# mit-acl/dpgo_ros

Measured on AMD Instinct MI355X. Metric: ms/RBCD-iteration + iterations-to-1e-6-relcost, sphere2500 5-agent, lower is better.
Workload: dtype f64; 1 GPU; sphere2500.g2o, 5 agents, synchronous round-robin RBCD, RGD(step 0.2, dense preconditioner) + Nesterov (restart 20), r=5, library weighting; mid-run iterations one launch each (k_step_fd: the private part of an agent's preconditioner product formed by the launch before its own, its row products by the one before that), hipGraphs of up to 256 iterations; agents=5, poses_per_agent=500, placement=agent a on rank a % N

## Files before the change

dpgo_ros_amd/capi.py:

```python
import ctypes as C
import os
import sys
import threading

import numpy as np

_HERE = os.path.dirname(os.path.abspath(__file__))
LIB_PATH = os.environ.get("DPGO_HIP_LIB") or os.path.join(_HERE, "libdpgo_hip.so")
_LIB = None


class Measurement(C.Structure):
    _fields_ = [("r1", C.c_int), ("p1", C.c_int), ("r2", C.c_int), ("p2", C.c_int),
                ("R", C.c_double * 9), ("t", C.c_double * 3),
                ("kappa", C.c_double), ("tau", C.c_double), ("weight", C.c_double),
                ("fixed_weight", C.c_int), ("is_known_inlier", C.c_int)]


MEAS_DTYPE = np.dtype([("r1", "<i4"), ("p1", "<i4"), ("r2", "<i4"), ("p2", "<i4"),
                       ("R", "<f8", (9,)), ("t", "<f8", (3,)),
                       ("kappa", "<f8"), ("tau", "<f8"), ("weight", "<f8"),
                       ("fixed_weight", "<i4"), ("is_known_inlier", "<i4")], align=True)
assert MEAS_DTYPE.itemsize == C.sizeof(Measurement)

# ... 818 lines not shown
    def iteration(self):
        return lib().dpgo_team_iteration(self.h)

    def cost(self):
        f = C.c_double()
        _chk(lib().dpgo_team_cost(self.h, C.byref(f)), "team_cost")
        return f.value

    def update_weights(self):
        return _chk(lib().dpgo_team_update_weights(self.h), "team_update_weights")

    def counters(self):
        out = np.zeros(11)
        lib().dpgo_team_get_counters(self.h, _d(out), 11)
        return out

    def stream(self):
        return lib().dpgo_team_stream(self.h)

    def time_kernel(self, agent_id, which, reps=200):
        ms, nbytes = C.c_double(), C.c_double()
        _chk(lib().dpgo_team_time_kernel(self.h, agent_id, which, reps, C.byref(ms), C.byref(nbytes)), "time_kernel")
        return ms.value, nbytes.value

    def global_X(self):
        return np.concatenate([self.agents[i].get_X() for i in self.ids])

    def certificate_apply(self, V, transport=None, owner_of_robot=None):
        N = int(sum(self.agents[i].n for i in self.ids))
        V = np.ascontiguousarray(V, dtype=np.float64).reshape(-1)
# ... 368 lines not shown
```

dpgo_ros_amd/csrc/capi.hip:

```cpp
#include <unistd.h>

#include <atomic>
#include <array>
#include <chrono>
#include <thread>
#include <unordered_map>

#include <mutex>
#include <random>
#include "certify_internal.h"
#include "team_internal.h"

using namespace dpgo;
using namespace dpgo_host;

extern "C" {

const char *dpgo_last_error(void) { return g_err.c_str(); }

void dpgo_default_params(dpgo_params_t *p, int r, int num_robots) {
  std::memset(p, 0, sizeof *p);
  p->d = 3; p->r = r; p->num_robots = num_robots;
  p->method = DPGO_METHOD_RTR;
  p->rgd_stepsize = 1e-3; p->rgd_use_preconditioner = 1;
// ... 77 lines not shown
    int cus = 0;
    if (hipDeviceGetAttribute(&cus, hipDeviceAttributeMultiprocessorCount, device) == hipSuccess) t->num_cus = cus;
    int lds = 0;
    if (hipDeviceGetAttribute(&lds, hipDeviceAttributeMaxSharedMemoryPerBlock, device) == hipSuccess && lds > 0) t->max_lds = lds;
    const char *e3 = std::getenv("DPGO_BAKE_SEL");
    if (e3) t->bake_sel = (e3[0] == '0') ? 0 : 1;
    const char *e4 = std::getenv("DPGO_BAKE_DESC");
    if (e4) t->bake_desc = (e4[0] == '0') ? 0 : 1;
    const char *e2 = std::getenv("DPGO_FUSED_RTR");
    if (e2) t->use_fused_rtr = (e2[0] == '0') ? 0 : 1;
    const char *e5 = std::getenv("DPGO_FUSED_EVAL");
    if (e5) t->use_fused_eval = (e5[0] == '0') ? 0 : 1;
    if (const char *e6 = std::getenv("DPGO_FE_MIN_N")) t->fe_min_n = std::max(32, std::atoi(e6));
    if (const char *e7 = std::getenv("DPGO_FE_CARRY")) t->use_fe_carry = (e7[0] == '0') ? 0 : 1;
    if (const char *e8 = std::getenv("DPGO_FE_DEEP")) t->use_fe_deep = (e8[0] == '0') ? 0 : 1;
    if (const char *e10 = std::getenv("DPGO_REPORT_TAIL")) t->use_report_tail = (e10[0] == '0') ? 0 : 1;
    if (const char *e11 = std::getenv("DPGO_REPORT_PREFETCH")) t->prefetch_reports = (e11[0] == '0') ? 0 : 1;
    if (t->d_nest_all.alloc(3 * std::max(1, num_local)) ||
        hipMemset(t->d_nest_all.p, 0, sizeof(NestState) * 3 * std::max(1, num_local)) != hipSuccess) {
      delete t; set_err("hand-off state allocation failed"); return nullptr;
    }
    *t->h_bar_err = 0;
  }
  for (int k = 0; k < num_local; ++k) {
    auto a = std::make_unique<Agent>();
    a->id = agent_ids[k]; a->local = k; a->mu = p->gnc_init_mu;
    t->id2local[a->id] = k;
    t->ag.push_back(std::move(a));
  }
  return t;
// ... 1318 lines not shown
    auto sel_at = [&](int rep) { return t->sched[(size_t)((it0 + rep) % P)]; };
    NestState *nest_own = t->d_nest_all.p, *nest_fe[2] = {t->d_nest_all.p + na, t->d_nest_all.p + 2 * na};
    launch_nest_pre(cc, SEL_SCHED, -1, na, mn, p.num_robots, p.restart_interval, 1);
    const int total_reps = ((reps + 1) & ~1) + 8;
    reps = total_reps - 8;
    const int fd_m0 = fe_deep_m0(t);
    if (fd_m0 > 0) {
      int nblk_all = 0;
      for (auto &b : t->ag) nblk_all = std::max(nblk_all, (4 * b->n + 7) / 8);
      double *pacc[2] = {t->d_fd_pacc.p, t->d_fd_pacc.p + (size_t)nblk_all * p.r * 256};
      const int s0 = sel_at(0), s1 = sel_at(1), s2 = sel_at(2);
      launch_fd_prime(cc, s0, s1, s2, mn, p.num_robots, p.restart_interval, nest_own);
      launch_fd_open(cc, fd_m0, s0, s1, pacc[0]);
      for (int k = 0; k < total_reps; ++k) {
        if (k == 8) HIPC(hipEventRecord(e0, t->stream));
        const int flags = FD_IN | (k + 1 < total_reps ? FD_P : 0) | (k + 2 < total_reps ? FD_W : 0) | (k + 3 < total_reps ? FD_Y : 0);
        launch_step_fd(cc, fd_m0, sel_at(k), sel_at(k + 1), sel_at(k + 2), sel_at(k + 3), p.rgd_stepsize, p.num_robots,
                       p.restart_interval, k == 0 ? nest_own : nest_fe[k & 1], nest_fe[(k + 1) & 1], k & 1, flags,
                       pacc[k & 1], pacc[(k + 1) & 1]);
      }
    } else
    for (int k = 0; k < total_reps; ++k) {
      if (k == 8) HIPC(hipEventRecord(e0, t->stream));
      launch_step_fe(cc, sel_at(k), sel_at(k + 1), p.rgd_stepsize, p.num_robots, p.restart_interval,
                     k == 0 ? nest_own : nest_fe[k & 1], nest_fe[(k + 1) & 1], k & 1, sel_at(k + 2),
                     fe_carry_flags(t, k, total_reps, it0));
    }
    HIPC(hipEventRecord(e1, t->stream));
    launch_eval_stats(cc, mn, 0, 0, 1, p.num_robots, p.restart_interval, SEL_SCHED, sel_at(total_reps - 1), nest_fe[total_reps & 1]);
    HIPC(hipEventSynchronize(e1));
    HIPC(hipStreamSynchronize(t->stream));
    t->iter += total_reps;
    float ms = 0;
// ... 48 lines not shown
```

dpgo_ros_amd/csrc/dpgo_dev.h:

```cpp
#pragma once
#include <hip/hip_runtime.h>

namespace dpgo {

enum Buf {
  B_X = 0, B_XPREV, B_Y, B_V, B_G,
  B_EGRAD, B_GF, B_Z, B_ETA, B_R0, B_R1, B_D0, B_D1, B_HD,
  B_X2, B_EGRAD2, B_GF2, B_HETA, B_T0, B_T1, B_T2,
  B_XALT, B_ALTPAD_, B_YALT,
  NBUF
};
constexpr int B_CARRY_Y = B_R0, B_CARRY_W = B_R1, B_CARRY_X = B_D0;
constexpr int B_CARRY_G = B_D1;
constexpr int FE_CARRY_IN = 1, FE_CARRY_W = 2, FE_CARRY_Y = 4;
constexpr int FE_MAX_EDGES = 160;
constexpr int B_ALT = B_XALT - B_X;
static_assert(B_YALT - B_Y == B_ALT, "X and Y twins share one displacement");

struct SharedEdgeDev {
  int lpose;
  int slot;
  int src_agent_local;
  int src_frame;
  int src_robot, pad_;
// ... 89 lines not shown
constexpr int PART_C = 2 * MAX_PART * PART_STRIDE;
constexpr int PART_D = 3 * MAX_PART * PART_STRIDE;
constexpr int PART_E = 4 * MAX_PART * PART_STRIDE;
constexpr int PART_TOTAL = 5 * MAX_PART * PART_STRIDE;

constexpr int LOOKAHEAD_MAX_AGENTS = 8;

struct FeBases {
  const double *ybase[LOOKAHEAD_MAX_AGENTS];
  int npose[LOOKAHEAD_MAX_AGENTS];
  double *part[LOOKAHEAD_MAX_AGENTS];
};

constexpr int FD_IN = 1, FD_P = 2, FD_W = 4, FD_Y = 8;
constexpr int FD_STATS = 16, FD_LASTAT = 32;
struct FdNext {
  const double *Md;
  const double *Gd;
  int N4d, nblk_d;
  unsigned char ord_d[32];
  int n_e, soa_w_e, npub_e, pad_;
  const int *soa_col_e;
  const double *soa_val_e;
  const int *pub_index_e;
  const double *Ye;
  double *We, *Xe, *Ge;
  unsigned char ord_e[32];
};

struct TeamDev {
// ... 25 lines not shown
```

dpgo_ros_amd/csrc/kernels.h:

```cpp
#pragma once
#include <hip/hip_runtime.h>
#include "dpgo_dev.h"

namespace dpgo {

struct LaunchCtx {
  int r;
  hipStream_t stream;
  const AgentDev *agents;
  TeamDev *team;
  int ny = 1;
  int dense_max_n = 1 << 30;
  bool any_two_level = false;
  int tl_max_wg = 0;
  const int *host_precond = nullptr;
  const AgentDev *host_agents = nullptr;
  int num_agents = 0;
  bool bake_desc = false;
  const int *up_slots = nullptr;
  const double *up_in = nullptr;
  int up_n0 = 0, up_n1 = 0;
  int max_lds = 160 * 1024;
  int stage_cap = 0;
  const NestState *nest_all = nullptr;
// ... 31 lines not shown
size_t eval_staged_lds_bytes(int r, int cap);
constexpr int EVS_STATIC_LDS = 8 * 1024;
void launch_hess(const LaunchCtx &c, int sel, int max_n, int xb, int egb, int vb, int ob, int poff);
void launch_precond(const LaunchCtx &c, int sel, int max_n, int mode, int xb, int vb, int zb, int sp, int max_inner,
                    double step, int accel, int num_robots, int advance = PADV_NONE, int restart_interval = 1, int ahead = 0);
void launch_eval_stats(const LaunchCtx &c, int max_n, int first, int has_eval, int has_stats, int num_robots,
                       int restart_interval, int eval_sel = SEL_SCHED, int stats_sel = SEL_SCHED, const NestState *nest_copy = nullptr);
bool step_fe_supported(int r);
int step_fe_max_edges();
void launch_step_fe(const LaunchCtx &c, int sel, int next_sel, double step, int num_robots, int restart_interval,
                    const NestState *nest_src, NestState *nest_dst, int parity, int next2_sel = -1, int carry = 0);
int step_fe_carry_max_poses();
int step_fd_pick_m0(int min_private_chunks);
void launch_fd_open(const LaunchCtx &c, int m0, int s0, int s1, double *pacc_out);
void launch_fd_prime(const LaunchCtx &c, int s0, int s1, int s2, int max_n, int num_robots, int restart_interval, const NestState *nest_src);
void launch_step_fd(const LaunchCtx &c, int m0, int sel, int next_sel, int next2_sel, int next3_sel, double step, int num_robots,
                    int restart_interval, const NestState *nest_src, NestState *nest_dst, int parity, int flags,
                    const double *pacc_in, double *pacc_out);
constexpr int LS_MAX_TRIALS = 8;
void launch_ls_trials(const LaunchCtx &c, int sel, int max_n, int dirb, double step0, double shrink, int ntrials);
void launch_ls_cost(const LaunchCtx &c, int sel, int max_n, int dirb, int ntrials);
void launch_ls_apply(const LaunchCtx &c, int sel, int max_n, double step0, double shrink, double sigma, int ntrials, int tail = 0,
                     int num_robots = 1, int restart_interval = 1);
void launch_tcg_hv(const LaunchCtx &c, int sel, int max_n, int sp, int max_inner);
void launch_retract(const LaunchCtx &c, int sel, int max_n, int xb, int eb, double scale, int ob, int guard_state);
void launch_project_raw(const LaunchCtx &c, const double *X, double *out, int n);
void launch_tangent_raw(const LaunchCtx &c, const double *X, const double *V, double *out, int n);
void launch_retract_raw(const LaunchCtx &c, const double *X, const double *E, double *out, int n);
void launch_nest_pre(const LaunchCtx &c, int sel, int only_agent, int num_agents, int max_n, int num_robots,
                     int restart_interval, int fused_restart = 0);
void launch_stats_nest(const LaunchCtx &c, int num_agents, int max_n, int num_robots, int restart_interval);
void launch_nest_post(const LaunchCtx &c, int sel, int max_n, int num_robots, int restart_interval);
// ... 66 lines not shown
```

dpgo_ros_amd/csrc/step_deep.hip:

```cpp
#include "kernel_common.h"
#include <algorithm>

namespace dpgo {

constexpr int FD_KC = 2048;
#ifndef DPGO_FD_HEAD
#define DPGO_FD_HEAD 0
#endif
#ifndef DPGO_FD_GC_LATE
#define DPGO_FD_GC_LATE 0
#endif
#ifndef DPGO_FD_PACC_WT
#define DPGO_FD_PACC_WT 0
#endif
#ifndef DPGO_FD_E_EARLY
#define DPGO_FD_E_EARLY 0
#endif
#ifndef DPGO_FD_KA_PREFETCH
#define DPGO_FD_KA_PREFETCH 1
#endif
constexpr int FD_HEAD = DPGO_FD_HEAD;

enum { FD_SY_C = 0, FD_SY_E, FD_SY_D, FD_SY_F, FD_SY_N, FD_SY_RQ, FD_SY_COUNT = 8 };

// ... 19 lines not shown
template <int R>
__device__ __forceinline__ int fd_pos_off(const unsigned char *ord, int pose) {
  const int ch = pose >> 4;
  int p = 0;
#pragma unroll
  for (int i = 0; i < 32; ++i) p = ((int)ord[i] == ch) ? i : p;
  return p * 64 * R + (pose & 15) * 4 * R;
}

template <int R>
struct FdXn {
  double2 v[3][2 * R];
};

template <int R>
__device__ __forceinline__ void fd_xn_request(const AgentDev &ag, const FeBases &fb, int parity, int ln, FdXn<R> &xr) {
#pragma unroll
  for (int q = 0; q < 3; ++q) {
    {
      unsigned wsel = 0;
#pragma unroll
      for (int k = 0; k < 32; ++k) {
        const unsigned wk = ag.fe_code[(32 * q + k < FE_MAX_EDGES / 2) ? 32 * q + k : FE_MAX_EDGES / 2 - 1];
        wsel = ((ln >> 1) == k) ? wk : wsel;
      }
      const unsigned code = (ln & 1) ? (wsel >> 16) : (wsel & 0xffffu);
      const int sa = (int)(code >> 12), sf = (int)(code & 0xfffu);
      const double *yb = fb.ybase[0];
      int yn = fb.npose[0];
#pragma unroll
      for (int k = 1; k < LOOKAHEAD_MAX_AGENTS; ++k) { yb = (sa == k) ? fb.ybase[k] : yb; yn = (sa == k) ? fb.npose[k] : yn; }
      const double *xp = yb + (parity ? (size_t)B_ALT * 4 * R * yn : (size_t)0) + (size_t)sf * 4 * R;
#pragma unroll
      for (int k = 0; k < 2 * R; ++k) xr.v[q][k] = ld2(xp + 2 * k);
    }
  }
}

template <int R>
__device__ __forceinline__ void fd_xn_to_lds(const AgentDev &ag, int ln, const FdXn<R> &xr, double *Es) {
  constexpr int EPE = 4 * R + 16;
  int nsh = ag.nshared;
  asm volatile("" : "+v"(nsh));
#pragma unroll
  for (int q = 0; q < 3; ++q) {
    if (64 * q < nsh && 64 * q + ln < nsh) {
      double *E = Es + (size_t)(64 * q + ln) * EPE;
#pragma unroll
      for (int k = 0; k < 2 * R; ++k) *reinterpret_cast<double2 *>(E + 2 * k) = xr.v[q][k];
    }
  }
}

struct FdCf {
  static constexpr int TRIPS = FE_MAX_EDGES * 8 / 64;
  double2 v[TRIPS];
};

__device__ __forceinline__ void fd_cf_request(const AgentDev &ag, int ln, FdCf &cr) {
  const int nit = ag.nshared * 8;
#pragma unroll
  for (int j = 0; j < FdCf::TRIPS; ++j) cr.v[j] = ld2(ag.fe_coef + 2 * min(64 * j + ln, nit - 1));
}

// ... 21 lines not shown
  o.restart_next = ((ns.iter + 3) % restart_interval) == 0;
  o.restart_next2 = ((ns.iter + 4) % restart_interval) == 0;
  o.restart_next3 = ((ns.iter + 5) % restart_interval) == 0;
  o.nest_gamma = o.restart_now ? 0.0 : (1.0 + sqrt(1.0 + 4.0 * Nr * Nr * ns.gamma * ns.gamma)) / (2.0 * Nr);
  const double g2 = (1.0 + sqrt(1.0 + 4.0 * Nr * Nr * o.nest_gamma * o.nest_gamma)) / (2.0 * Nr);
  o.ahead_alpha = 1.0 / (g2 * Nr);
  const double gamma_next = o.restart_next ? 0.0 : g2;
  const double g3 = (1.0 + sqrt(1.0 + 4.0 * Nr * Nr * gamma_next * gamma_next)) / (2.0 * Nr);
  o.ahead2_alpha = 1.0 / (g3 * Nr);
  const double gamma_next2 = o.restart_next2 ? 0.0 : g3;
  const double g4 = (1.0 + sqrt(1.0 + 4.0 * Nr * Nr * gamma_next2 * gamma_next2)) / (2.0 * Nr);
  o.ahead3_alpha = 1.0 / (g4 * Nr);
  return o;
}

template <int R, int NC>
struct FdCur {
  double2 mc[NC];
  double pa[R];
};

template <int R, int M0, int NC>
__device__ __forceinline__ void fd_cur_request(const AgentDev &ag, const double *pacc_in, int bx, int nblk, int l, FdCur<R, NC> &cu) {
  const int cg = (l >> 5) & 7, kl = l & 31;
  const int N4 = ag.N4, col = 8 * bx + cg;
  const double *Mc = ag.M + (size_t)((col < N4) ? col : 0) * N4;
#pragma unroll
  for (int i = 0; i < NC; ++i) cu.mc[i] = ld2_nt(Mc + min(2 * kl + 64 * (int)ag.fe_ord[M0 + i], N4 - 2));
#pragma unroll
  for (int a = 0; a < R; ++a) cu.pa[a] = gp(pacc_in)[((size_t)min(bx, nblk - 1) * R + a) * 256 + l];
// ... 37 lines not shown
#elif defined(DPGO_FD_ENDS)
#define FD_TRACE_DECL
#define FD_STAMP(k) do { if ((k) == 0 && blockIdx.x == 100 && threadIdx.x == 256) ag.part[PART_E + 4000 * PART_STRIDE + 64] = (double)wall_clock64(); } while (0)
#define FD_FLUSH() do { if (blockIdx.x == 100 && (threadIdx.x & 63) == 0) ag.part[PART_E + 4000 * PART_STRIDE + (threadIdx.x >> 6) * 16 + 15] = (double)wall_clock64(); } while (0)
#else
#define FD_TRACE_DECL
#define FD_STAMP(k) do { } while (0)
#define FD_FLUSH() do { } while (0)
#endif

template <int R, int M0>
__global__ __launch_bounds__(512) void k_step_fd(TeamDev *team, int sel, int next_sel, double step, int num_robots, int restart_interval,
                                                 const NestState *nest_src, NestState *nest_dst, int parity, const AgentDev agv,
                                                 int next3_sel, int flags, const FdNext nx, const FeBases fb,
                                                 const double *__restrict__ pacc_in, double *__restrict__ pacc_out, int nblk_all,
                                                 int num_agents) {
  const AgentDev &ag = agv;
#if DPGO_FD_KA_PREFETCH
  {
    const unsigned *ka = (const unsigned *)__builtin_amdgcn_kernarg_segment_ptr();
    constexpr int KA_LINES = (int)((sizeof(AgentDev) + sizeof(FdNext) + sizeof(FeBases) + 160 + 63) / 64);
    unsigned touch = 0;
#pragma unroll
    for (int i = 0; i < KA_LINES; ++i) touch |= ka[16 * i];
    asm volatile("" ::"s"(touch));
  }
#endif
  const double *__restrict__ Xr = ag.buf[parity ? B_XALT : B_X];
  const double *__restrict__ Yr = ag.buf[parity ? B_YALT : B_Y];
  double *__restrict__ Xw = ag.buf[parity ? B_X : B_XALT];
  double *__restrict__ Yw = ag.buf[parity ? B_Y : B_YALT];
// ... 233 lines not shown
    }
    fd_wait(&sy[FD_SY_F], 4);
    if (ln < 8 * R) {
      double s = 0;
#pragma unroll
      for (int q = 0; q < 32; ++q) s += red[q * (8 * R + 1) + ln];
      zs[ln] = s;
    }
    FD_STAMP(6);
    WSYNC();
    const FdNest nn = fd_nest(ns, num_robots, restart_interval);
    const bool restart_now = nn.restart_now, restart_next = nn.restart_next;
    const double nest_gamma = nn.nest_gamma, ahead_alpha = nn.ahead_alpha;
    const bool ahead_opt = next_sel == sel;
    const bool stats = in && (flags & FD_STATS) != 0, lastat = in && (flags & FD_LASTAT) != 0;
    if (ln < 2) tl_rel[ln] = 0.0;
    {
      const int lp = ln >> 4, s = ln & 15;
      if (lp < npose) {
        const size_t o = (size_t)(lp ? pj1 : pj0) * 4 * R;
        double *xs = tl_x + lp * 4 * R, *vsv = tl_v + lp * 4 * R, *ys = tl_y + lp * 4 * R, *Ss = tl_s + lp * 16;
        double *zz = zs + lp * 4 * R;
        const double *x0 = Ysh + lp * 4 * R, *v0 = Esh[0] + lp * 4 * R, *y0 = Esh[1] + lp * 4 * R;
        const int i0 = s, i1 = s + 16;
        const bool h0 = i0 < 4 * R, h1 = i1 < 4 * R;
        tangent_lanes<R>(x0, zz, Ss, s);
        if (h0) xs[i0] = x0[i0] - step * zz[i0];
        if (h1) xs[i1] = x0[i1] - step * zz[i1];
        lanes_sync();
        qf_lanes<R>(xs, Ss, s);
// ... 30 lines not shown
          if (h0 && in) {
            Xw[o + i0] = xs[i0];
            if (!ahead_opt) { Yw[o + i0] = xs[i0]; vsv[i0] = xs[i0]; }
            else Yw[o + i0] = reset ? xs[i0] : y0[i0];
          }
          if (h1 && in) {
            Xw[o + i1] = xs[i1];
            if (!ahead_opt) { Yw[o + i1] = xs[i1]; vsv[i1] = xs[i1]; }
            else Yw[o + i1] = reset ? xs[i1] : y0[i1];
          }
          if (lastat && !ahead_opt && s == 0) gp(ag.part)[PART_D + (lp ? pj1 : pj0)] = 0.0;
        } else {
          if (h0) ys[i0] = (1.0 - ahead_alpha) * xs[i0] + ahead_alpha * vsv[i0];
          if (h1) ys[i1] = (1.0 - ahead_alpha) * xs[i1] + ahead_alpha * vsv[i1];
          lanes_sync();
          polar_lanes<R>(ys, Ss, s);
          FD_STAMP(9);
          if (h0 && in) { Yw[o + i0] = ys[i0]; Xw[o + i0] = ys[i0]; }
          if (h1 && in) { Yw[o + i1] = ys[i1]; Xw[o + i1] = ys[i1]; }
          if (lastat && !ahead_opt && s == 0) {
            double rel2 = 0;
#pragma unroll
            for (int i = 0; i < 4 * R; ++i) { const double d = ys[i] - xs[i]; rel2 += d * d; }
            gp(ag.part)[PART_D + (lp ? pj1 : pj0)] = rel2;
          }
        }
        lanes_sync();
        if (h0 && in) ag.buf[B_V][o + i0] = vsv[i0];
        if (h1 && in) ag.buf[B_V][o + i1] = vsv[i1];
      }
    }
    if (stats) {
      WSYNC();
      double rl = (ln < npose) ? tl_rel[ln] : 0.0;
      rl = wave_sum(rl);
      if (ln == 0 && own) gp(ag.part)[PART_B + (size_t)bx * PART_STRIDE + 2] = rl;
    }
    FD_STAMP(15);
    FD_FLUSH();
    return;
  }

  const int h = cwv - 6;
  if (h == 0) {
    FdXn<R> er;
    fd_xn_request<R>(ag, fb, parity, ln, er);
    FD_STAMP(9);
    FdCur<R, NC> cu;
    fd_cur_request<R, M0, NC>(ag, pacc_in, bx, nblk, tid - 256, cu);
    FD_STAMP(10);
    fd_signal_requested(&sy[FD_SY_RQ]);
    FD_STAMP(11);
    __builtin_amdgcn_s_setprio(3);
    fd_xn_to_lds<R>(ag, ln, er, Es);
    fd_signal(&sy[FD_SY_E]);
    FD_STAMP(8);
    fd_wait(&sy[FD_SY_D], 2);
    fd_cur_product<R, M0, NC>(cu, vs, red, tid - 256);
    fd_signal(&sy[FD_SY_F]);
    if (bx == 0 && ln < LOOKAHEAD_MAX_AGENTS && in) {
      const int k = ln;
      const double Nr = (double)num_robots;
      if (k < num_agents) {
        NestState s2 = nest_src[k];
        const bool restart = ((s2.iter + 2) % restart_interval) == 0;
        if (restart) { s2.gamma = 0; s2.alpha = 0; }
        else {
          s2.gamma = (1.0 + sqrt(1.0 + 4.0 * Nr * Nr * s2.gamma * s2.gamma)) / (2.0 * Nr);
          s2.alpha = 1.0 / (s2.gamma * Nr);
// ... 47 lines not shown
    double *yp = const_cast<double *>(ya);
    double *xa = yp - (size_t)(B_Y - B_X) * vlen, *va = yp + (size_t)(B_V - B_Y) * vlen;
    const size_t da = (size_t)B_ALT * vlen;
    const double *xr = parity ? xa + da : xa, *yr = parity ? yp + da : yp;
    double *oX = parity ? xa : xa + da, *oY = parity ? yp : yp + da, *oV = va;
    const int la_pose = gq - lo;
    const bool la_opt = next_sel == a;
    const size_t o = (size_t)la_pose * 4 * R;
    double la_x[4 * R], la_v[4 * R];
#pragma unroll
    for (int i = 0; i < 2 * R; ++i) {
      const double2 tx = ld2(xr + o + 2 * i), tv = ld2(va + o + 2 * i);
      la_x[2 * i] = tx.x; la_x[2 * i + 1] = tx.y; la_v[2 * i] = tv.x; la_v[2 * i + 1] = tv.y;
    }
    const NestState ns = nest_src[sel];
    FD_STAMP(10);
    fd_signal_requested(&sy[FD_SY_RQ]);
    FD_STAMP(11);
    __builtin_amdgcn_s_setprio(3);
#if !DPGO_FD_E_EARLY
    fd_cf_to_lds<R>(ag, ln, er, Es);
    fd_signal(&sy[FD_SY_E]);
    FD_STAMP(8);
#endif
    fd_wait(&sy[FD_SY_D], 2);
    fd_cur_product<R, M0, NC>(cu, vs, red, tid - 256);
    fd_signal(&sy[FD_SY_F]);
    __builtin_amdgcn_s_setprio(0);
    const FdNest nn = fd_nest(ns, num_robots, restart_interval);
    if (lact) {
      const bool st = in, lastat = in && (flags & FD_LASTAT) != 0;
      double *pa_ = fb.part[0];
#pragma unroll
      for (int k = 1; k < LOOKAHEAD_MAX_AGENTS; ++k) pa_ = (a == k) ? fb.part[k] : pa_;
      if (lastat) {
        double *xprev = yp - (size_t)(B_Y - B_XPREV) * vlen;
#pragma unroll
        for (int i = 0; i < 4 * R; ++i) gp(xprev)[o + i] = la_x[i];
      }
      if (nn.restart_next) {
#pragma unroll
        for (int i = 0; i < 4 * R; ++i) {
          if (st) oX[o + i] = la_x[i];
          if (!la_opt) { if (st) { oY[o + i] = la_x[i]; oV[o + i] = la_x[i]; } la_v[i] = la_x[i]; }
          else if (st) oY[o + i] = yr[o + i];
        }
// ... 193 lines not shown
  int nblk_all = 0;
  for (int k = 0; k < c.num_agents; ++k) nblk_all = std::max(nblk_all, (c.host_agents[k].N4 + 7) / 8);
  const int gridp = ((c.host_agents[s0].N4 + 7) / 8 + 7) / 8 * 8;
  if (m0 != 24) return;
  switch (c.r) {
    case 3: hipLaunchKernelGGL((k_fd_rows<3>), dim3(nblk_all, 2), dim3(64), 0, c.stream, c.agents, s0, s1, nblk_all);
            hipLaunchKernelGGL((k_fd_partial<3, 24>), dim3(gridp), dim3(256), 0, c.stream, c.agents, s0, pacc_out); break;
    case 4: hipLaunchKernelGGL((k_fd_rows<4>), dim3(nblk_all, 2), dim3(64), 0, c.stream, c.agents, s0, s1, nblk_all);
            hipLaunchKernelGGL((k_fd_partial<4, 24>), dim3(gridp), dim3(256), 0, c.stream, c.agents, s0, pacc_out); break;
    case 5: hipLaunchKernelGGL((k_fd_rows<5>), dim3(nblk_all, 2), dim3(64), 0, c.stream, c.agents, s0, s1, nblk_all);
            hipLaunchKernelGGL((k_fd_partial<5, 24>), dim3(gridp), dim3(256), 0, c.stream, c.agents, s0, pacc_out); break;
    default: break;
  }
}

void launch_step_fd(const LaunchCtx &c, int m0, int sel, int next_sel, int next2_sel, int next3_sel, double step, int num_robots,
                    int restart_interval, const NestState *nest_src, NestState *nest_dst, int parity, int flags,
                    const double *pacc_in, double *pacc_out) {
  const AgentDev &d = c.host_agents[sel], &dd = c.host_agents[next_sel], &de = c.host_agents[next2_sel];
  int nblk_all = 0;
  for (int k = 0; k < c.num_agents; ++k) nblk_all = std::max(nblk_all, (c.host_agents[k].N4 + 7) / 8);
  const int grid = (nblk_all + 7) / 8 * 8;
  FeBases fb = {};
  for (int k = 0; k < c.num_agents && k < LOOKAHEAD_MAX_AGENTS; ++k) { fb.ybase[k] = c.host_agents[k].buf[B_Y]; fb.npose[k] = c.host_agents[k].n; fb.part[k] = c.host_agents[k].part; }
  FdNext nx = {};
  nx.Md = dd.M; nx.N4d = dd.N4; nx.nblk_d = (dd.N4 + 7) / 8; nx.Gd = dd.buf[B_CARRY_G];
  for (int i = 0; i < 32; ++i) { nx.ord_d[i] = dd.fe_ord[i]; nx.ord_e[i] = de.fe_ord[i]; }
  nx.n_e = de.n; nx.soa_w_e = de.soa_w; nx.npub_e = de.npub; nx.soa_col_e = de.soa_col; nx.soa_val_e = de.soa_val;
  nx.pub_index_e = de.pub_index; nx.Ye = de.buf[B_CARRY_Y]; nx.We = de.buf[B_CARRY_W]; nx.Xe = de.buf[B_CARRY_X]; nx.Ge = de.buf[B_CARRY_G];
#define FD_LAUNCH(RR, MM)                                                                                                   \
  hipLaunchKernelGGL((k_step_fd<RR, MM>), dim3(grid), dim3(512), 0, c.stream, c.team, sel, next_sel, step, num_robots,        \
                     restart_interval, nest_src, nest_dst, parity, d, next3_sel, flags, nx, fb, pacc_in, pacc_out, nblk_all, \
                     c.num_agents)
#define FD_LAUNCH_M(RR)                                   \
  switch (m0) {                                           \
    case 24: FD_LAUNCH(RR, 24); break;                    \
    default: break;                                       \
  }
  switch (c.r) {
    case 3: FD_LAUNCH_M(3); break;
    case 4: FD_LAUNCH_M(4); break;
    case 5: FD_LAUNCH_M(5); break;
    default: break;
  }
#undef FD_LAUNCH_M
#undef FD_LAUNCH
}

// ... 2 lines not shown
```

dpgo_ros_amd/csrc/team_internal.h:

```cpp
#pragma once
#include <hip/hip_runtime.h>

#include <algorithm>
#include <chrono>
#include <cmath>
#include <cstdio>
#include <cstring>
#include <functional>
#include <map>
#include <memory>
#include <string>
#include <tuple>
#include <utility>
#include <vector>

#include "../../include/dpgo_hip.h"
#include "dpgo_dev.h"
#include "kernels.h"
#include "twolevel.h"

namespace dpgo_host {
using namespace dpgo;

inline thread_local std::string g_err;
// ... 83 lines not shown
    return 0;
  }
};

enum StatusSrc {
  REL_NEVER = -1,
  REL_TILES_D = 0,
  REL_FUSED_B = 1,
  REL_NONE = 2,
  REL_POSE_D = 4,
  REL_TILES_E = 5,
};

enum Counter {
  CNT_PRECOND = 0, CNT_PRECOND_BYTES, CNT_EVALS, CNT_EVAL_BYTES, CNT_ITERATIONS, CNT_REPORT_WAIT_US, CNT_REPORTS,
  CNT_ONE_LAUNCH, CNT_CARRIED, CNT_DEEP, CNT_REPORT_TAILS, CNT_COUNT
};
static_assert(CNT_ITERATIONS == 4 && CNT_ONE_LAUNCH == 7 && CNT_REPORT_TAILS == 10 && CNT_COUNT == 11, "positions are part of the C-ABI");

constexpr int PHASE_WHOLE = 0, PHASE_BEGIN = 1, PHASE_END = 2;

struct Agent {
  int id = 0, local = 0;
  std::vector<dpgo_measurement_t> odom, priv, shared;
  bool index_dirty = true, data_dirty = true;
  bool struct_uploaded = false;
  int n = 0;
  int max_pose_edges = 0, max_tile_edges = 0;
  std::vector<std::pair<int, int>> np;
  std::vector<char> np_has[2];
  std::vector<int> neighbors;
  int state = DPGO_WAIT_FOR_DATA;
  int iter = 0, instance = 0;
// ... 107 lines not shown
  std::map<int, hipGraphExec_t> graphs;
  std::map<int, int> graph_flip;
  bool graph_valid = false;
  double counters[dpgo_host::CNT_COUNT] = {};
  struct Peer { double *base = nullptr; size_t off_x = 0, off_y = 0; int n = 0; };
  std::map<int, Peer> peers;
  dpgo_host::DevBuf<unsigned long long> d_mail;
  bool mail_finegrained = false;
  std::map<int, unsigned long long *> peer_mail;
  std::vector<void *> mail_handles;
  std::vector<unsigned long long> last_fin;
  dpgo_host::DevBuf<dpgo::NestState> d_nest_all;
  int use_fused_eval = 1;
  int use_fe_carry = 1;
  int use_fe_deep = 1;
  int prefetch_reports = 1;
  int use_report_tail = 1;
  dpgo_host::DevBuf<double> d_fd_pacc;
  int fe_min_n = 0;
  struct SharedLink { dpgo_measurement_t *from, *to; int to_local; };
  std::vector<SharedLink> shared_links;
  std::vector<std::pair<const void *, size_t>> shared_links_key;
  dpgo_host::PinnedBuf<double> h_resid;
  struct PendingUpload { const int *slots = nullptr; const double *in = nullptr; int n0 = 0, n1 = 0; } pend_up;
  struct ReportOffer { bool valid = false, taken = false; dpgo::ReportTail rt; } rep_offer;
  int *h_bar_err = nullptr;
  int num_cus = 0;
  int max_lds = 160 * 1024;
  int dense_max_n = 0;
  std::vector<int> precond_of;
// ... 71 lines not shown
std::vector<int> public_ids(const Agent &a, int nbr);
std::vector<int> neighbor_ids(const Agent &a, int nbr);
int finalize_agent(dpgo_team *t, Agent &a, double *scratch);
int sync_descs(dpgo_team *t);
int sync_descs_noflush(dpgo_team *t);
int flush_stage(dpgo_team *t);
int stage_to_pinned(dpgo_team *t, Agent &a, int *n0, int *n1);

inline int local_or_remote(const dpgo_team *t, int robot) { auto it = t->id2local.find(robot); return it == t->id2local.end() ? SEL_REMOTE : it->second; }
inline bool restart_due(const dpgo_team *t) { return t->prm.acceleration && ((t->iter + 2) % t->prm.restart_interval) == 0; }

void drop_graphs(dpgo_team *t);
int check_exchange_error(dpgo_team *t);
int ensure_mailbox(dpgo_team *t);
bool fused_eval_eligible(dpgo_team *t);
int fe_deep_m0(dpgo_team *t);
int fe_carry_flags(dpgo_team *t, int rep, int nfe, int iter0);

int check_joined_to_pose0(const dpgo_measurement_t *m, int nm, int n, const char *what);

bool acquire_fused_rtr_lock(dpgo_team *t);
void release_fused_rtr_lock(dpgo_team *t);
double converged_ratio(const Agent &a);
void mark_optimized(dpgo_team *t, Agent &a, int rel_src, bool success);
struct OptFlags {
  int aux = 0, pull = 0;
  bool capture = false, fused = false, last_advances = false;
  int rtr_tail = 0;
  int ls_tail = 0;
  bool skip_stats = false;
// ... 23 lines not shown
```

dpgo_ros_amd/csrc/team_run.hip:

```cpp
#include "team_internal.h"

using namespace dpgo;
using namespace dpgo_host;

namespace dpgo_host {

void drop_graphs(dpgo_team *t) {
  for (auto &kv : t->graphs) if (kv.second) (void)hipGraphExecDestroy(kv.second);
  t->graphs.clear();
  t->graph_flip.clear();
}

int check_exchange_error(dpgo_team *t) {
  if (!t->h_bar_err || !*t->h_bar_err) return 0;
  const int code = *t->h_bar_err;
  *t->h_bar_err = 0;
  drop_graphs(t);
  set_err("an in-kernel exchange timed out (code " + std::to_string(code) + ": 2 hand-off of the one-launch RTR solve, 3 two-level "
          "preconditioner, 4 mailbox of the device-side UPDATE token): the iterates since the last successful synchronisation are invalid");
  return DPGO_ERR;
}

static void revalidate_graphs(dpgo_team *t) { if (!t->graph_valid) { drop_graphs(t); t->graph_valid = true; } }

// ... 116 lines not shown
  int L;
  int nfe;
  bool deep;
};

static RunWindow make_window(const RunPlan &pl, bool lead, int B, int iter0) {
  RunWindow w{};
  w.lead = lead; w.B = B; w.iter0 = iter0;
  w.fe = pl.fe_ok && (pl.fd_m0 > 0 ? B >= 6 : B > pl.P + 2);
  w.L = std::min(B, pl.P);
  w.deep = w.fe && pl.fd_m0 > 0 && ((B - 1) & ~1) >= 4;
  w.nfe = !w.fe ? 0 : (w.deep ? (B - 1) & ~1 : std::max(0, B - w.L - 1) & ~1);
  return w;
}

static void enqueue_fe_deep(dpgo_team *t, const LaunchCtx &c, int m0, const RunWindow &w, NestState *nest_own, NestState *const nest_fe[2]) {
  const dpgo_params_t &p = t->prm;
  const int nfe = w.nfe, B = w.B, L = w.L;
  auto sel_at = [&](int rep) { return agent_at(t, w.iter0 + rep); };
  int nblk_all = 0;
  for (auto &a : t->ag) nblk_all = std::max(nblk_all, (4 * a->n + 7) / 8);
  double *pacc[2] = {t->d_fd_pacc.p, t->d_fd_pacc.p + (size_t)nblk_all * p.r * 256};
  const int s0 = sel_at(0), s1 = sel_at(1), s2 = sel_at(2);
  launch_fd_prime(c, s0, s1, s2, t->max_n, p.num_robots, p.restart_interval, nest_own);
  launch_fd_open(c, m0, s0, s1, pacc[0]);
  for (int rep = 0; rep < nfe; ++rep) {
    const int flags = FD_IN | (rep + 1 < nfe ? FD_P : 0) | (rep + 2 < nfe ? FD_W : 0) | (rep + 3 < nfe ? FD_Y : 0) |
                      (rep >= B - L ? FD_STATS : 0) | ((rep + 1 < B && rep + 1 >= B - L) ? FD_LASTAT : 0);
    launch_step_fd(c, m0, sel_at(rep), sel_at(rep + 1), sel_at(rep + 2), sel_at(rep + 3), p.rgd_stepsize, p.num_robots,
                   p.restart_interval, rep == 0 ? nest_own : nest_fe[rep & 1], nest_fe[(rep + 1) & 1], rep & 1, flags,
                   pacc[rep & 1], pacc[(rep + 1) & 1]);
  }
}

static int enqueue_window(dpgo_team *t, const RunPlan &pl, const RunWindow &w) {
  const dpgo_params_t &p = t->prm;
  const int B = w.B, na = (int)t->ag.size(), mn = t->max_n;
  auto sel_at = [&](int rep) { return pl.bake ? agent_at(t, w.iter0 + rep) : SEL_SCHED; };
  if (w.lead) {
    const int rc = enqueue_team_iteration(t, true, true, SEL_SCHED, PHASE_WHOLE);
    if (rc) return rc;
  }
  if (B > 0 && p.acceleration && pl.pipelined) {
    LaunchCtx c = t->ctx();
    c.bake_desc = pl.bake && t->bake_desc;
    launch_nest_pre(c, SEL_SCHED, -1, na, mn, p.num_robots, p.restart_interval, 1);
// ... 31 lines not shown
  }
  return 0;
}

static int window_graph(dpgo_team *t, const RunPlan &pl, const RunWindow &w, hipGraphExec_t *out) {
  const int phase = pl.bake ? w.iter0 % pl.P : -1;
  const int base = ((((w.lead ? 1 : 0) + 2 * w.B) * 16 + phase + 1) * 2 + (w.fe ? 1 : 0)) * 2;
  const int key = base + (t->graph_flip[base / 2] ^= 1);
  return graph_for_key(t, key, true, [&] { return enqueue_window(t, pl, w); }, out);
}

static void account_window(dpgo_team *t, const RunPlan &pl, const RunWindow &w) {
  const dpgo_params_t &p = t->prm;
  const int lead = w.lead ? 1 : 0, batch = w.B + lead;
  t->counters[CNT_ONE_LAUNCH] += w.nfe;
  if (w.deep) { t->counters[CNT_CARRIED] += w.nfe; t->counters[CNT_DEEP] += w.nfe; }
  else for (int q = 0; q < w.nfe; ++q) t->counters[CNT_CARRIED] += (fe_carry_flags(t, q, w.nfe, w.iter0) & FE_CARRY_IN) ? 1 : 0;
  for (auto &a : t->ag) a->rel_src = p.acceleration ? ((pl.pipelined && w.B >= 2) ? REL_POSE_D : REL_TILES_D) : REL_NONE;
  for (int q = 0; q < batch; ++q) {
    const bool is_lead = w.lead && q == 0;
    Agent &a = *t->ag[agent_at(t, w.iter0 + q)];
    const int evals = pl.ls ? 2 + (ls_trials(p) + 3) / 4 : ((!is_lead && q - lead < w.nfe) ? 1 : 2);
    count_work(t, a, 1, evals);
    if (is_lead) count_work(t, a, 1, evals);
    mark_optimized(t, a, (is_lead || pl.ls) ? REL_TILES_E : REL_FUSED_B, true);
    if (q == batch - 1) {
      a.opt_pending_rgd = true;
      a.rel_src = (w.B > 0 && !pl.ls) ? REL_FUSED_B : REL_TILES_D;
    }
  }
}
// ... 239 lines not shown
```

Before: 12.94 us.

## Defer Nesterov lookahead polar projection to the next step_fd launch

Skips the polar retraction of the Nesterov lookahead Y in the current k_step_fd launch and has the following launch project the previous agent's rows when it loads them, both into LDS for the neighbour exchange and in the lookahead path. This removes the projection from the critical path of the producing launch and overlaps it with the consumer's loads. In exchange the consumer does extra polar work and needs prev_sel threaded through. Correctness depends on the restart-interval and lastat edge cases that the code excludes.

```diff
diff --git a/dpgo_ros_amd/capi.py b/dpgo_ros_amd/capi.py
--- a/dpgo_ros_amd/capi.py
+++ b/dpgo_ros_amd/capi.py
@@ -856,6 +856,11 @@
         out = np.zeros(11)
         lib().dpgo_team_get_counters(self.h, _d(out), 11)
         return out
+
+    def deferred_launches(self):
+        out = np.zeros(12)
+        lib().dpgo_team_get_counters(self.h, _d(out), 12)
+        return int(out[11])
 
     def stream(self):
         return lib().dpgo_team_stream(self.h)
diff --git a/dpgo_ros_amd/csrc/capi.hip b/dpgo_ros_amd/csrc/capi.hip
--- a/dpgo_ros_amd/csrc/capi.hip
+++ b/dpgo_ros_amd/csrc/capi.hip
@@ -115,6 +115,7 @@
     if (const char *e6 = std::getenv("DPGO_FE_MIN_N")) t->fe_min_n = std::max(32, std::atoi(e6));
     if (const char *e7 = std::getenv("DPGO_FE_CARRY")) t->use_fe_carry = (e7[0] == '0') ? 0 : 1;
     if (const char *e8 = std::getenv("DPGO_FE_DEEP")) t->use_fe_deep = (e8[0] == '0') ? 0 : 1;
+    if (const char *e9 = std::getenv("DPGO_FD_DEFER")) t->use_fd_defer = (e9[0] == '0') ? 0 : 1;
     if (const char *e10 = std::getenv("DPGO_REPORT_TAIL")) t->use_report_tail = (e10[0] == '0') ? 0 : 1;
     if (const char *e11 = std::getenv("DPGO_REPORT_PREFETCH")) t->prefetch_reports = (e11[0] == '0') ? 0 : 1;
     if (t->d_nest_all.alloc(3 * std::max(1, num_local)) ||
@@ -1463,9 +1464,10 @@
       launch_fd_open(cc, fd_m0, s0, s1, pacc[0]);
       for (int k = 0; k < total_reps; ++k) {
         if (k == 8) HIPC(hipEventRecord(e0, t->stream));
-        const int flags = FD_IN | (k + 1 < total_reps ? FD_P : 0) | (k + 2 < total_reps ? FD_W : 0) | (k + 3 < total_reps ? FD_Y : 0);
-        launch_step_fd(cc, fd_m0, sel_at(k), sel_at(k + 1), sel_at(k + 2), sel_at(k + 3), p.rgd_stepsize, p.num_robots,
-                       p.restart_interval, k == 0 ? nest_own : nest_fe[k & 1], nest_fe[(k + 1) & 1], k & 1, flags,
+        const int flags = FD_IN | (k + 1 < total_reps ? FD_P : 0) | (k + 2 < total_reps ? FD_W : 0) | (k + 3 < total_reps ? FD_Y : 0) |
+                          fd_defer_bits(t->use_fd_defer != 0, k, total_reps, false, false);
+        launch_step_fd(cc, fd_m0, sel_at(k > 0 ? k - 1 : 0), sel_at(k), sel_at(k + 1), sel_at(k + 2), sel_at(k + 3), p.rgd_stepsize,
+                       p.num_robots, p.restart_interval, k == 0 ? nest_own : nest_fe[k & 1], nest_fe[(k + 1) & 1], k & 1, flags,
                        pacc[k & 1], pacc[(k + 1) & 1]);
       }
     } else
diff --git a/dpgo_ros_amd/csrc/dpgo_dev.h b/dpgo_ros_amd/csrc/dpgo_dev.h
--- a/dpgo_ros_amd/csrc/dpgo_dev.h
+++ b/dpgo_ros_amd/csrc/dpgo_dev.h
@@ -127,6 +127,7 @@
 
 constexpr int FD_IN = 1, FD_P = 2, FD_W = 4, FD_Y = 8;
 constexpr int FD_STATS = 16, FD_LASTAT = 32;
+constexpr int FD_DEFER = 64, FD_PREV_DEFER = 128;
 struct FdNext {
   const double *Md;
   const double *Gd;
diff --git a/dpgo_ros_amd/csrc/kernels.h b/dpgo_ros_amd/csrc/kernels.h
--- a/dpgo_ros_amd/csrc/kernels.h
+++ b/dpgo_ros_amd/csrc/kernels.h
@@ -69,8 +69,8 @@
 int step_fd_pick_m0(int min_private_chunks);
 void launch_fd_open(const LaunchCtx &c, int m0, int s0, int s1, double *pacc_out);
 void launch_fd_prime(const LaunchCtx &c, int s0, int s1, int s2, int max_n, int num_robots, int restart_interval, const NestState *nest_src);
-void launch_step_fd(const LaunchCtx &c, int m0, int sel, int next_sel, int next2_sel, int next3_sel, double step, int num_robots,
-                    int restart_interval, const NestState *nest_src, NestState *nest_dst, int parity, int flags,
+void launch_step_fd(const LaunchCtx &c, int m0, int prev_sel, int sel, int next_sel, int next2_sel, int next3_sel, double step,
+                    int num_robots, int restart_interval, const NestState *nest_src, NestState *nest_dst, int parity, int flags,
                     const double *pacc_in, double *pacc_out);
 constexpr int LS_MAX_TRIALS = 8;
 void launch_ls_trials(const LaunchCtx &c, int sel, int max_n, int dirb, double step0, double shrink, int ntrials);
diff --git a/dpgo_ros_amd/csrc/step_deep.hip b/dpgo_ros_amd/csrc/step_deep.hip
--- a/dpgo_ros_amd/csrc/step_deep.hip
+++ b/dpgo_ros_amd/csrc/step_deep.hip
@@ -57,7 +57,8 @@
 };
 
 template <int R>
-__device__ __forceinline__ void fd_xn_request(const AgentDev &ag, const FeBases &fb, int parity, int ln, FdXn<R> &xr) {
+__device__ __forceinline__ int fd_xn_request(const AgentDev &ag, const FeBases &fb, int parity, int ln, FdXn<R> &xr, int who) {
+  int from_who = 0;
 #pragma unroll
   for (int q = 0; q < 3; ++q) {
     {
@@ -69,6 +70,7 @@
       }
       const unsigned code = (ln & 1) ? (wsel >> 16) : (wsel & 0xffffu);
       const int sa = (int)(code >> 12), sf = (int)(code & 0xfffu);
+      from_who |= (sa == who) ? (1 << q) : 0;
       const double *yb = fb.ybase[0];
       int yn = fb.npose[0];
 #pragma unroll
@@ -78,6 +80,7 @@
       for (int k = 0; k < 2 * R; ++k) xr.v[q][k] = ld2(xp + 2 * k);
     }
   }
+  return from_who;
 }
 
 template <int R>
@@ -91,6 +94,27 @@
       double *E = Es + (size_t)(64 * q + ln) * EPE;
 #pragma unroll
       for (int k = 0; k < 2 * R; ++k) *reinterpret_cast<double2 *>(E + 2 * k) = xr.v[q][k];
+    }
+  }
+}
+
+template <int R>
+__device__ __forceinline__ void fd_xn_project(const AgentDev &ag, int ln, int from_who, double *Es) {
+  constexpr int EPE = 4 * R + 16;
+  int nsh = ag.nshared;
+  asm volatile("" : "+v"(nsh));
+#pragma unroll 1
+  for (int q = 0; q < 3; ++q) {
+    const bool mine = ((from_who >> q) & 1) && 64 * q + ln < nsh;
+    if (__builtin_amdgcn_ballot_w64(mine) == 0) continue;
+    if (mine) {
+      double *E = Es + (size_t)(64 * q + ln) * EPE;
+      double a[3 * R];
+#pragma unroll
+      for (int i = 0; i < 3 * R; ++i) a[i] = E[i];
+      polar_inplace<R>(a);
+#pragma unroll
+      for (int i = 0; i < 3 * R; ++i) E[i] = a[i];
     }
   }
 }
@@ -142,6 +166,10 @@
   return o;
 }
 
+__device__ __forceinline__ bool fd_prev_deferred(int flags, int prev_iter, int restart_interval) {
+  return (flags & FD_PREV_DEFER) != 0 && ((prev_iter + 2) % restart_interval) != 0;
+}
+
 template <int R, int NC>
 struct FdCur {
   double2 mc[NC];
@@ -209,7 +237,7 @@
                                                  const NestState *nest_src, NestState *nest_dst, int parity, const AgentDev agv,
                                                  int next3_sel, int flags, const FdNext nx, const FeBases fb,
                                                  const double *__restrict__ pacc_in, double *__restrict__ pacc_out, int nblk_all,
-                                                 int num_agents) {
+                                                 int num_agents, int prev_sel) {
   const AgentDev &ag = agv;
 #if DPGO_FD_KA_PREFETCH
   {
@@ -473,6 +501,7 @@
     const double nest_gamma = nn.nest_gamma, ahead_alpha = nn.ahead_alpha;
     const bool ahead_opt = next_sel == sel;
     const bool stats = in && (flags & FD_STATS) != 0, lastat = in && (flags & FD_LASTAT) != 0;
+    const bool defer = in && (flags & FD_DEFER) != 0 && !lastat && !ahead_opt;
     if (ln < 2) tl_rel[ln] = 0.0;
     {
       const int lp = ln >> 4, s = ln & 15;
@@ -533,7 +562,7 @@
           if (h0) ys[i0] = (1.0 - ahead_alpha) * xs[i0] + ahead_alpha * vsv[i0];
           if (h1) ys[i1] = (1.0 - ahead_alpha) * xs[i1] + ahead_alpha * vsv[i1];
           lanes_sync();
-          polar_lanes<R>(ys, Ss, s);
+          if (!defer) polar_lanes<R>(ys, Ss, s);
           FD_STAMP(9);
           if (h0 && in) { Yw[o + i0] = ys[i0]; Xw[o + i0] = ys[i0]; }
           if (h1 && in) { Yw[o + i1] = ys[i1]; Xw[o + i1] = ys[i1]; }
@@ -563,7 +592,8 @@
   const int h = cwv - 6;
   if (h == 0) {
     FdXn<R> er;
-    fd_xn_request<R>(ag, fb, parity, ln, er);
+    const int from_prev = fd_xn_request<R>(ag, fb, parity, ln, er, prev_sel);
+    const int prev_iter = nest_src[(flags & FD_PREV_DEFER) ? prev_sel : sel].iter;
     FD_STAMP(9);
     FdCur<R, NC> cu;
     fd_cur_request<R, M0, NC>(ag, pacc_in, bx, nblk, tid - 256, cu);
@@ -572,6 +602,7 @@
     FD_STAMP(11);
     __builtin_amdgcn_s_setprio(3);
     fd_xn_to_lds<R>(ag, ln, er, Es);
+    if (fd_prev_deferred(flags, prev_iter, restart_interval)) fd_xn_project<R>(ag, ln, from_prev, Es);
     fd_signal(&sy[FD_SY_E]);
     FD_STAMP(8);
     fd_wait(&sy[FD_SY_D], 2);
@@ -649,6 +680,7 @@
       la_x[2 * i] = tx.x; la_x[2 * i + 1] = tx.y; la_v[2 * i] = tv.x; la_v[2 * i + 1] = tv.y;
     }
     const NestState ns = nest_src[sel];
+    const int prev_iter = nest_src[(flags & FD_PREV_DEFER) ? prev_sel : sel].iter;
     FD_STAMP(10);
     fd_signal_requested(&sy[FD_SY_RQ]);
     FD_STAMP(11);
@@ -665,6 +697,7 @@
     const FdNest nn = fd_nest(ns, num_robots, restart_interval);
     if (lact) {
       const bool st = in, lastat = in && (flags & FD_LASTAT) != 0;
+      if (a == prev_sel && fd_prev_deferred(flags, prev_iter, restart_interval)) polar_inplace<R>(la_x);
       double *pa_ = fb.part[0];
 #pragma unroll
       for (int k = 1; k < LOOKAHEAD_MAX_AGENTS; ++k) pa_ = (a == k) ? fb.part[k] : pa_;
@@ -888,8 +921,8 @@
   }
 }
 
-void launch_step_fd(const LaunchCtx &c, int m0, int sel, int next_sel, int next2_sel, int next3_sel, double step, int num_robots,
-                    int restart_interval, const NestState *nest_src, NestState *nest_dst, int parity, int flags,
+void launch_step_fd(const LaunchCtx &c, int m0, int prev_sel, int sel, int next_sel, int next2_sel, int next3_sel, double step,
+                    int num_robots, int restart_interval, const NestState *nest_src, NestState *nest_dst, int parity, int flags,
                     const double *pacc_in, double *pacc_out) {
   const AgentDev &d = c.host_agents[sel], &dd = c.host_agents[next_sel], &de = c.host_agents[next2_sel];
   int nblk_all = 0;
@@ -905,7 +938,7 @@
 #define FD_LAUNCH(RR, MM)                                                                                                   \
   hipLaunchKernelGGL((k_step_fd<RR, MM>), dim3(grid), dim3(512), 0, c.stream, c.team, sel, next_sel, step, num_robots,        \
                      restart_interval, nest_src, nest_dst, parity, d, next3_sel, flags, nx, fb, pacc_in, pacc_out, nblk_all, \
-                     c.num_agents)
+                     c.num_agents, prev_sel)
 #define FD_LAUNCH_M(RR)                                   \
   switch (m0) {                                           \
     case 24: FD_LAUNCH(RR, 24); break;                    \
diff --git a/dpgo_ros_amd/csrc/team_internal.h b/dpgo_ros_amd/csrc/team_internal.h
--- a/dpgo_ros_amd/csrc/team_internal.h
+++ b/dpgo_ros_amd/csrc/team_internal.h
@@ -121,9 +121,10 @@
 
 enum Counter {
   CNT_PRECOND = 0, CNT_PRECOND_BYTES, CNT_EVALS, CNT_EVAL_BYTES, CNT_ITERATIONS, CNT_REPORT_WAIT_US, CNT_REPORTS,
-  CNT_ONE_LAUNCH, CNT_CARRIED, CNT_DEEP, CNT_REPORT_TAILS, CNT_COUNT
-};
-static_assert(CNT_ITERATIONS == 4 && CNT_ONE_LAUNCH == 7 && CNT_REPORT_TAILS == 10 && CNT_COUNT == 11, "positions are part of the C-ABI");
+  CNT_ONE_LAUNCH, CNT_CARRIED, CNT_DEEP, CNT_REPORT_TAILS, CNT_DEFERRED, CNT_COUNT
+};
+static_assert(CNT_ITERATIONS == 4 && CNT_ONE_LAUNCH == 7 && CNT_REPORT_TAILS == 10 && CNT_DEFERRED == 11 && CNT_COUNT == 12,
+              "positions are part of the C-ABI");
 
 constexpr int PHASE_WHOLE = 0, PHASE_BEGIN = 1, PHASE_END = 2;
 
@@ -261,6 +262,7 @@
   int use_fused_eval = 1;
   int use_fe_carry = 1;
   int use_fe_deep = 1;
+  int use_fd_defer = 1;
   int prefetch_reports = 1;
   int use_report_tail = 1;
   dpgo_host::DevBuf<double> d_fd_pacc;
@@ -362,6 +364,10 @@
 int check_exchange_error(dpgo_team *t);
 int ensure_mailbox(dpgo_team *t);
 bool fused_eval_eligible(dpgo_team *t);
+inline int fd_defer_bits(bool on, int rep, int nfe, bool lastat, bool prev_lastat) {
+  if (!on) return 0;
+  return ((rep + 1 < nfe && !lastat) ? FD_DEFER : 0) | ((rep > 0 && !prev_lastat) ? FD_PREV_DEFER : 0);
+}
 int fe_deep_m0(dpgo_team *t);
 int fe_carry_flags(dpgo_team *t, int rep, int nfe, int iter0);
 
diff --git a/dpgo_ros_amd/csrc/team_run.hip b/dpgo_ros_amd/csrc/team_run.hip
--- a/dpgo_ros_amd/csrc/team_run.hip
+++ b/dpgo_ros_amd/csrc/team_run.hip
@@ -154,9 +154,17 @@
   return w;
 }
 
+static int fd_window_flags(const dpgo_team *t, const RunWindow &w, int rep) {
+  const int nfe = w.nfe, B = w.B, L = w.L;
+  auto lastat = [&](int q) { return q + 1 < B && q + 1 >= B - L; };
+  return FD_IN | (rep + 1 < nfe ? FD_P : 0) | (rep + 2 < nfe ? FD_W : 0) | (rep + 3 < nfe ? FD_Y : 0) |
+         (rep >= B - L ? FD_STATS : 0) | (lastat(rep) ? FD_LASTAT : 0) |
+         fd_defer_bits(t->use_fd_defer != 0, rep, nfe, lastat(rep), rep > 0 && lastat(rep - 1));
+}
+
 static void enqueue_fe_deep(dpgo_team *t, const LaunchCtx &c, int m0, const RunWindow &w, NestState *nest_own, NestState *const nest_fe[2]) {
   const dpgo_params_t &p = t->prm;
-  const int nfe = w.nfe, B = w.B, L = w.L;
+  const int nfe = w.nfe;
   auto sel_at = [&](int rep) { return agent_at(t, w.iter0 + rep); };
   int nblk_all = 0;
   for (auto &a : t->ag) nblk_all = std::max(nblk_all, (4 * a->n + 7) / 8);
@@ -165,11 +173,9 @@
   launch_fd_prime(c, s0, s1, s2, t->max_n, p.num_robots, p.restart_interval, nest_own);
   launch_fd_open(c, m0, s0, s1, pacc[0]);
   for (int rep = 0; rep < nfe; ++rep) {
-    const int flags = FD_IN | (rep + 1 < nfe ? FD_P : 0) | (rep + 2 < nfe ? FD_W : 0) | (rep + 3 < nfe ? FD_Y : 0) |
-                      (rep >= B - L ? FD_STATS : 0) | ((rep + 1 < B && rep + 1 >= B - L) ? FD_LASTAT : 0);
-    launch_step_fd(c, m0, sel_at(rep), sel_at(rep + 1), sel_at(rep + 2), sel_at(rep + 3), p.rgd_stepsize, p.num_robots,
-                   p.restart_interval, rep == 0 ? nest_own : nest_fe[rep & 1], nest_fe[(rep + 1) & 1], rep & 1, flags,
-                   pacc[rep & 1], pacc[(rep + 1) & 1]);
+    launch_step_fd(c, m0, sel_at(rep > 0 ? rep - 1 : 0), sel_at(rep), sel_at(rep + 1), sel_at(rep + 2), sel_at(rep + 3),
+                   p.rgd_stepsize, p.num_robots, p.restart_interval, rep == 0 ? nest_own : nest_fe[rep & 1],
+                   nest_fe[(rep + 1) & 1], rep & 1, fd_window_flags(t, w, rep), pacc[rep & 1], pacc[(rep + 1) & 1]);
   }
 }
 
@@ -231,7 +237,10 @@
   const dpgo_params_t &p = t->prm;
   const int lead = w.lead ? 1 : 0, batch = w.B + lead;
   t->counters[CNT_ONE_LAUNCH] += w.nfe;
-  if (w.deep) { t->counters[CNT_CARRIED] += w.nfe; t->counters[CNT_DEEP] += w.nfe; }
+  if (w.deep) {
+    t->counters[CNT_CARRIED] += w.nfe; t->counters[CNT_DEEP] += w.nfe;
+    for (int q = 0; q < w.nfe; ++q) t->counters[CNT_DEFERRED] += (fd_window_flags(t, w, q) & FD_DEFER) ? 1 : 0;
+  }
   else for (int q = 0; q < w.nfe; ++q) t->counters[CNT_CARRIED] += (fe_carry_flags(t, q, w.nfe, w.iter0) & FE_CARRY_IN) ? 1 : 0;
   for (auto &a : t->ag) a->rel_src = p.acceleration ? ((pl.pipelined && w.B >= 2) ? REL_POSE_D : REL_TILES_D) : REL_NONE;
   for (int q = 0; q < batch; ++q) {
```

After: 13.29 us. 1.03x slower.
